# noahpieta/bedops

Measured on AMD Instinct MI355X. Metric: intervals/sec, bedops --intersect 100M×100M BED3 at 1/2/4/8 MI355X, higher is better.
Workload: dtype int64; 1 GPU; bedops --intersect A.bed B.bed: BED3 text in HBM -> parse -> merge -> intersect -> BED text in HBM; parallelism=single GPU, output_rows=38507974

## Files before the change

bedops_amd/csrc/bg_load.hip:

```cpp
#include <algorithm>
#include <cstring>
#include <map>

#include <type_traits>

#include "bg_internal.h"
#include "bg_parse.h"
#include "bg_strtod.h"

#define TT 8192
#define HB 16
#define HA 256
#define LBUF (HB + TT + HA + 32)
#define LCAP 1536
#define REC_CAP (1u << 20)

__device__ __forceinline__ uint32_t nl_mask4(uint32_t w) {
  uint32_t x = w ^ 0x0A0A0A0Au;
  uint32_t nz = ((x & 0x7F7F7F7Fu) + 0x7F7F7F7Fu) | x;
  return ~nz & 0x80808080u;
}

__device__ __forceinline__ uint4 load16(const uint8_t* __restrict__ txt, int64_t base,
                                        uint64_t nbytes) {
// ... 822 lines not shown
    const uint64_t r = r0 + k;
    int64_t key = LLONG_MIN;
    const int64_t le = (k + 1 < L) ? t0 + lst[k + 1] - 1 : last_end;
    if (r < nrows && le >= 0) {
      Fast F;
      const uint32_t run = (rl == rh) ? rl : run_of(R, ls, rl, rh);
      const RunInfo& I = R.info[run];
      double sc = 0;
      if (parse_line_fast(buf, wsm, dgm, lst[k], (uint32_t)(le - ls), F, I.tlen <= 8) &&
          F.toklen == I.tlen && F.tlo == I.tlo && F.thi == I.thi &&
          (kind != BG_BED5 ||
           parse_score_fast(buf, wsm, dgm, lst[k], (uint32_t)(le - ls), F.rest, sc))) {
        emit_row(R, run, ls, r, F.start, F.end, KS, KE, st, key, mlen);
        if (rest_off) {
          rest_off[r] = (uint64_t)(ls + F.rest);
          rest_len[r] = (uint32_t)(le - ls - F.rest);
        }
        if (score) score[r] = sc;
      } else {
        key = PENDING;
      }
    }
    lkey[k] = key;
  }
  for (uint32_t k = threadIdx.x; k < L; k += BG_NT) {
    if (lkey[k] != PENDING) continue;
    lkey[k] = LLONG_MIN;
    const int64_t ls = t0 + lst[k];
    const uint64_t r = r0 + k;
    const int64_t le = (k + 1 < L) ? t0 + lst[k + 1] - 1 : last_end;
    Line Ln;
    parse_line_slow(T, ls, le, kind, Ln);
    if (Ln.err) {
      if (Ln.err == ERR_BLANK) atomicAdd(&st->nblank, 1ULL);
      bg_report(st, r, Ln.err);
      KS[r] = KE[r] = 0;
      continue;
    }
    const uint32_t run = (rl == rh) ? rl : run_of(R, ls, rl, rh);
    if (Ln.hash != R.info[run].hash) {
      bg_report(st, r, ERR_UNSORTED);
      continue;
    }
    int64_t key;
    emit_row(R, run, ls, r, Ln.start, Ln.end, KS, KE, st, key, mlen);
    lkey[k] = key;
    if (rest_off) {
      rest_off[r] = (uint64_t)Ln.rest;
      rest_len[r] = (uint32_t)(le - Ln.rest);
    }
    if (score) {
      score[r] = Ln.score;
      if (Ln.scoreint <= 0) atomicOr(&st->flags, 1ULL);
      if (Ln.scoreint < 0) big_push(st, big, bigcap, r, Ln.spos);
    }
  }
#pragma unroll
  for (int d = 32; d >= 1; d >>= 1) mlen = max(mlen, (int64_t)__shfl_xor(mlen, d, 64));
  if (bg_lane() == 0 && mlen > *(volatile long long*)&st->maxlen) atomicMax(&st->maxlen, (long long)mlen);
  __syncthreads();
  for (uint32_t k = threadIdx.x + 1; k < L; k += BG_NT)
    if (lkey[k] != LLONG_MIN && lkey[k - 1] != LLONG_MIN && lkey[k] < lkey[k - 1])
      bg_report(st, r0 + k, ERR_UNSORTED);
}

__global__ void k_check_bounds(const int64_t* __restrict__ KS, const uint64_t* __restrict__ row0,
                               uint32_t ntiles, uint64_t nrows, bg_dstatus* st) {
  const uint32_t t = blockIdx.x * blockDim.x + threadIdx.x;
  if (t >= ntiles) return;
  const uint64_t r = row0[t];
  for (uint64_t q = r; q < r + 2 && q < nrows; ++q)
    if (q > 0 && KS[q] < KS[q - 1]) bg_report(st, q, ERR_UNSORTED);
}

struct SetTiles {
  int64_t* tmax;
  int64_t* tlast;
  uint64_t* base;
  uint64_t* nloc;
  uint32_t* absorbed;
  uint64_t* nrow;
  int64_t* gb;
};
__device__ __forceinline__ int64_t set_key(const int64_t* X, uint64_t b, int64_t gb, uint64_t i) {
  return gb >= 0 ? (gb | (int64_t)reinterpret_cast<const uint32_t*>(X + b)[i]) : X[b + i];
}

template <bool ONE = false, bool WSO = false, typename BufT = ParseBuf>
__device__ __forceinline__ bool set_row(const BufT& B, const uint16_t* lst, const TileText& T,
                                        const RunTable& R, uint32_t rl, uint32_t rh, int64_t t0,
                                        uint32_t k, uint32_t L, int64_t last_end, int64_t& ks,
                                        int64_t& ke, bg_dstatus* st) {
  const int64_t ls = t0 + lst[k];
  const int64_t le = (k + 1 < L) ? t0 + lst[k + 1] - 1 : last_end;
  if (le < 0) return false;
  const uint32_t run = ONE ? rl : ((rl == rh) ? rl : run_of(R, ls, rl, rh));
  const RunInfo& I = R.info[run];
  uint64_t start, end;
  Fast F;
  bool fast;
  if constexpr (WSO) fast = parse_line_fast_ws(B.buf, B.wsm, lst[k], (uint32_t)(le - ls), F, I.tlen <= 8);
  else fast = parse_line_fast(B.buf, B.wsm, B.dgm, lst[k], (uint32_t)(le - ls), F, I.tlen <= 8);
  if (fast && F.toklen == I.tlen && F.tlo == I.tlo && F.thi == I.thi) {
    start = F.start;
    end = F.end;
  } else {
    Line Ln;
    parse_line_slow(T, ls, le, BG_BED3, Ln);
    if (Ln.err) {
      bg_report(st, 0, Ln.err);
      return false;
    }
    if (Ln.hash != I.hash) {
      bg_report(st, 0, ERR_UNSORTED);
      return false;
    }
    start = Ln.start;
    end = Ln.end;
  }
  if (end > BG_KEY_COORD_MAX || start > end) bg_report(st, 0, ERR_RANGE);
  if (start == end) atomicOr(&st->flags, 2ULL);
  const int64_t g = (int64_t)I.gid << BG_KEY_SHIFT;
  ks = g | (int64_t)(start & BG_COORD_MASK);
  ke = g | (int64_t)(end & BG_COORD_MASK);
  return true;
}

template <int CTRL, int RMASK, bool BC>
__device__ __forceinline__ uint64_t dpp64(uint64_t v) {
  const int lo = __builtin_amdgcn_update_dpp(0, (int)(uint32_t)v, CTRL, RMASK, 0xF, BC);
  const int hi = __builtin_amdgcn_update_dpp(0, (int)(uint32_t)(v >> 32), CTRL, RMASK, 0xF, BC);
  return ((uint64_t)(uint32_t)hi << 32) | (uint32_t)lo;
}
__device__ __forceinline__ uint64_t wave_incl_max_u64(uint64_t v) {
  v = max(v, dpp64<0x111, 0xF, true>(v));
  v = max(v, dpp64<0x112, 0xF, true>(v));
  v = max(v, dpp64<0x114, 0xF, true>(v));
  v = max(v, dpp64<0x118, 0xF, true>(v));
  v = max(v, dpp64<0x142, 0xA, false>(v));
  v = max(v, dpp64<0x143, 0xC, false>(v));
  return v;
}
__device__ __forceinline__ uint64_t wave_shr1_u64(uint64_t v) { return dpp64<0x138, 0xF, true>(v); }

#define BG_SET_OVERFLOW 8ULL
#define BG_ROW_OVERFLOW 16ULL

__device__ __forceinline__ uint32_t wave_incl_max_u32(uint32_t v) {
  v = max(v, dpp32<0x111, 0xF, true>(v));
  v = max(v, dpp32<0x112, 0xF, true>(v));
  v = max(v, dpp32<0x114, 0xF, true>(v));
  v = max(v, dpp32<0x118, 0xF, true>(v));
  v = max(v, dpp32<0x142, 0xA, false>(v));
  v = max(v, dpp32<0x143, 0xC, false>(v));
  return v;
}
__device__ __forceinline__ uint32_t wave_incl_max_v(uint32_t v) { return wave_incl_max_u32(v); }
__device__ __forceinline__ uint64_t wave_incl_max_v(uint64_t v) { return wave_incl_max_u64(v); }
__device__ __forceinline__ uint32_t wave_shr1_v(uint32_t v) { return dpp32<0x138, 0xF, true>(v); }
__device__ __forceinline__ uint64_t wave_shr1_v(uint64_t v) { return wave_shr1_u64(v); }


__device__ __forceinline__ bool parse_score_fast_ws(const uint8_t* buf, const uint32_t* wsm, uint32_t q,
                                                    uint32_t len, uint32_t e1, double& score, bool& isint) {
  uint32_t WS = mask_window(wsm, q + e1);
  const uint32_t l2 = len - e1;
// ... 656 lines not shown
      if (SCORE) ok = ok && le - t0 <= TW + HA_R && score_fast_v(S, q, len, e1, sc);
    }
    if (ok) {
      if (start > end) bg_report(st, r, ERR_RANGE);
      if (start == end) atomicOr(&st->flags, 2ULL);
      mlen = max(mlen, (int64_t)end - (int64_t)start);
      if (ls == pos0) R.row[rl] = r;
      key = gbase | (int64_t)start;
      KS[r] = key;
      KE[r] = gbase | (int64_t)end;
      if (REST) {
        rest_off[r] = (uint64_t)(ls + e1);
        rest_len[r] = len - e1;
      }
      if (SCORE) {
        score[r] = sc;
        nonint |= !isint;
      }
    } else if (live) {
      row_line_general<REST, SCORE>(S, T, R, rl, rh, t0, q, ls, le, r, KS, KE, rest_off, rest_len, score, st,
                                    big, bigcap, key, mlen, nonint);
    }
    const int64_t pk = wave_shr1_i64(key);
    const int64_t prev = lane ? pk : carry;
    if (key != LLONG_MIN && prev != LLONG_MIN && key < prev) bg_report(st, r, ERR_UNSORTED);
    if (j == 0) kf = (int64_t)wave_readlane((uint64_t)key, 0);
    if (j + 1 == rounds) kl = (int64_t)wave_readlane((uint64_t)key, (int)(L - 1 - j * 64));
    carry = (int64_t)wave_readlane((uint64_t)key, 63);
  }
}

template <bool REST, bool SCORE>
__global__ void __launch_bounds__(128) __attribute__((amdgpu_waves_per_eu(6, 8))) k_parse_rv(
    const uint8_t* __restrict__ txt, uint64_t nb, uint64_t nrows, const uint64_t* __restrict__ row0,
    const uint32_t* __restrict__ runlo, const uint32_t* __restrict__ runhi, RunTable R,
    int64_t* __restrict__ KS, int64_t* __restrict__ KE, uint64_t* __restrict__ rest_off,
    uint32_t* __restrict__ rest_len, double* __restrict__ score, bg_dstatus* st, uint64_t* __restrict__ big,
    uint32_t bigcap) {
  __shared__ ParseLdsR SS[2];
  __shared__ uint32_t xl[2];
  __shared__ int64_t xk[2][2];
  const int lane = threadIdx.x & 63, h = __builtin_amdgcn_readfirstlane((int)(threadIdx.x >> 6));
  const uint32_t u = 2 * blockIdx.x + h;
  const int64_t t0 = (int64_t)u * TW;
  const bool inside = (uint64_t)t0 < nb;
  ParseLdsR& S = SS[h];
  int64_t last_end = -1;
  uint32_t L = 0;
  if (inside) {
    SubRegs V;
    load_sub<HA_R>(txt, nb, t0, V);
    L = prologue_v<ParseLdsR, LCAP_R, true, HA_R>(txt, nb, t0, V, S, last_end, st);
  }
  if (lane == 0) xl[h] = L;
  __syncthreads();
  const uint32_t L0 = xl[0];
  if (L0 > LCAP_R || xl[1] > LCAP_R) return;
  const int64_t tt = (int64_t)blockIdx.x * TT;
  const bool has0 = tt == 0 || SS[0].buf[HB - 1] == '\n';
  const uint64_t r0 = row0[blockIdx.x] + (has0 ? 0 : 1) + (h ? L0 : 0);
  int64_t mlen = 0, kf = LLONG_MIN, kl = LLONG_MIN;
  bool nonint = false;
  if (L > 0) {
    const TileText T{txt, S.buf, t0 - HB, t0 + TW + HA_R, nb};
    row_rounds_v<REST, SCORE>(S, T, R, runlo[u], runhi[u], t0, L, last_end, r0, nrows, KS, KE, rest_off,
                              rest_len, score, st, big, bigcap, kf, kl, mlen, nonint);
  }
  if (__ballot(nonint) && lane == 0) atomicOr(&st->flags, 1ULL);
#pragma unroll
  for (int d = 32; d >= 1; d >>= 1) mlen = max(mlen, (int64_t)__shfl_xor(mlen, d, 64));
  if (lane == 0 && mlen > *(volatile long long*)&st->maxlen) atomicMax(&st->maxlen, (long long)mlen);
  if (lane == 0) {
    xk[h][0] = kf;
    xk[h][1] = kl;
  }
  __syncthreads();
  if (h == 1 && lane == 0 && L0 > 0 && L > 0) {
    const int64_t a = xk[0][1], b = xk[1][0];
    if (a != LLONG_MIN && b != LLONG_MIN && b < a) bg_report(st, r0, ERR_UNSORTED);
  }
}


__global__ void __launch_bounds__(BG_NT) k_set_count(const int64_t* __restrict__ LCS, SetTiles TS,
                                                     const int64_t* __restrict__ mex,
                                                     uint32_t ntiles, uint64_t* __restrict__ cnt,
                                                     bg_dstatus* st, uint32_t u0) {
  __shared__ unsigned long long srows[BG_NT / 64];
  const uint32_t t = u0 + blockIdx.x * blockDim.x + threadIdx.x;
  uint64_t rows = 0;
  if (t < ntiles) {
    const uint64_t b = TS.base[t], n = TS.nloc[t];
    const int64_t gb = TS.gb[t];
    rows = TS.nrow[t];
    const int64_t first = n ? set_key(LCS, b, gb, 0) : 0;
    if (n > 0 && t > 0) {
      uint32_t u = t - 1;
      while (u > 0 && TS.tlast[u] == LLONG_MIN) --u;
      if (first < TS.tlast[u]) bg_report(st, 0, ERR_UNSORTED);
    }
    const int64_t M = mex[t];
    uint64_t a = 0;
    if (n && first <= M) {
      uint64_t step = 1;
      while (a + step < n && set_key(LCS, b, gb, a + step) <= M) {
        a += step;
        step <<= 1;
      }
      uint64_t lo = a + 1, hi = min(n, a + step);
      while (lo < hi) {
        const uint64_t mid = (lo + hi) >> 1;
        if (set_key(LCS, b, gb, mid) <= M) lo = mid + 1;
        else hi = mid;
      }
      a = lo;
    }
    TS.absorbed[t] = (uint32_t)a;
    cnt[t] = n - a;
  }
#pragma unroll
  for (int d = 32; d >= 1; d >>= 1) rows += __shfl_xor(rows, d, 64);
  if (bg_lane() == 0) srows[bg_wave()] = rows;
  __syncthreads();
  if (threadIdx.x == 0) {
    unsigned long long r = 0;
    for (int q = 0; q < BG_NT / 64; ++q) r += srows[q];
    if (r) atomicAdd((unsigned long long*)&st->pad[1], r);
  }
}

#define SW_TILES 64
__global__ void __launch_bounds__(BG_NT) k_set_write(const int64_t* __restrict__ LCS,
                                                     const int64_t* __restrict__ LCE, SetTiles TS,
                                                     const int64_t* __restrict__ mex,
                                                     const uint64_t* __restrict__ off,
                                                     uint32_t ntiles, int64_t* __restrict__ CS,
                                                     int64_t* __restrict__ CE, uint32_t u0, uint32_t nlast,
                                                     const uint64_t* __restrict__ carry,
                                                     unsigned long long* __restrict__ total_out) {
  __shared__ uint32_t cpre[SW_TILES + 1];
  __shared__ uint64_t src[SW_TILES], dst[SW_TILES];
  __shared__ uint32_t sab[SW_TILES];
  __shared__ int64_t sgb[SW_TILES];
  __shared__ int64_t first_end[SW_TILES];
  const uint32_t t0 = u0 + blockIdx.x * SW_TILES;
  const uint32_t nt = min((uint32_t)SW_TILES, ntiles - t0);
  const uint64_t cy = carry ? *carry : 0;
  uint32_t c = 0;
  if (threadIdx.x < nt) {
    const uint32_t t = t0 + threadIdx.x;
    const uint64_t b = TS.base[t], n = TS.nloc[t], a = TS.absorbed[t];
    const int64_t M = mex[t], gb = TS.gb[t];
    c = (uint32_t)(n - a);
    src[threadIdx.x] = b;
    sab[threadIdx.x] = (uint32_t)a;
    sgb[threadIdx.x] = gb;
    dst[threadIdx.x] = cy + off[t];
    first_end[threadIdx.x] = (c > 0) ? max(M, a > 0 ? set_key(LCE, b, gb, a - 1) : LLONG_MIN) : 0;
    if (t + 1 == nlast) {
      const uint64_t total = cy + off[t] + c;
      if (total > 0) CE[total - 1] = max(M, TS.tmax[t]);
      if (total_out) *total_out = total;
    }
  }
  if (threadIdx.x < 64) {
    const uint32_t inc = wave_incl_scan(c, OpSum());
    cpre[threadIdx.x + 1] = inc;
    if (threadIdx.x == 0) cpre[0] = 0;
  }
  __syncthreads();
  const uint32_t tot = cpre[nt];
  for (uint32_t e = threadIdx.x; e < tot; e += BG_NT) {
    uint32_t lo = 0, hi = nt - 1;
    while (lo < hi) {
      const uint32_t mid = (lo + hi + 1) >> 1;
      if (cpre[mid] <= e) lo = mid;
      else hi = mid - 1;
    }
    const uint32_t j = e - cpre[lo];
    const uint64_t g = dst[lo] + j, b = src[lo], i = sab[lo] + j;
    const int64_t gb = sgb[lo];
    CS[g] = set_key(LCS, b, gb, i);
    if (g > 0) CE[g - 1] = j == 0 ? first_end[lo] : set_key(LCE, b, gb, i - 1);
  }
}

constexpr uint32_t BK_T = 4096;

__global__ void __launch_bounds__(BG_NT) k_blank_marks(const uint8_t* __restrict__ txt, uint64_t nb,
                                                       uint32_t nt, int64_t* __restrict__ tnl,
                                                       int64_t* __restrict__ tns) {
  const uint32_t lane = threadIdx.x & 63, t = blockIdx.x * (BG_NT / 64) + (threadIdx.x >> 6);
  if (t >= nt) return;
  const uint64_t b0 = (uint64_t)t * BK_T + 64ull * lane;
  int64_t lnl = -1, lns = -2;
  for (uint32_t k = 0; k < 64 && b0 + k < nb; ++k) {
    const uint8_t ch = txt[b0 + k];
    if (ch == '\n') lnl = (int64_t)(b0 + k);
    else if (!bg_isws(ch)) lns = (int64_t)(b0 + k);
  }
  for (int d = 32; d >= 1; d >>= 1) {
    lnl = max(lnl, (int64_t)__shfl_xor(lnl, d, 64));
    lns = max(lns, (int64_t)__shfl_xor(lns, d, 64));
  }
  if (lane == 0) {
    tnl[t] = lnl;
    tns[t] = lns;
  }
}

__global__ void __launch_bounds__(BG_NT) k_blank_pack(const uint8_t* __restrict__ txt, uint64_t nb,
                                                      uint32_t nt, const int64_t* __restrict__ xnl,
                                                      const int64_t* __restrict__ xns,
                                                      uint64_t* __restrict__ cnt,
                                                      const uint64_t* __restrict__ off,
                                                      uint8_t* __restrict__ out) {
  const uint32_t lane = threadIdx.x & 63, t = blockIdx.x * (BG_NT / 64) + (threadIdx.x >> 6);
  if (t >= nt) return;
  const uint64_t b0 = (uint64_t)t * BK_T + 64ull * lane;
  int64_t lnl = -1, lns = -2;
  for (uint32_t k = 0; k < 64 && b0 + k < nb; ++k) {
    const uint8_t ch = txt[b0 + k];
    if (ch == '\n') lnl = (int64_t)(b0 + k);
    else if (!bg_isws(ch)) lns = (int64_t)(b0 + k);
  }
  for (int d = 1; d < 64; d <<= 1) {
    const int64_t a = __shfl_up(lnl, d, 64), b = __shfl_up(lns, d, 64);
    if (lane >= (uint32_t)d) {
      lnl = max(lnl, a);
      lns = max(lns, b);
    }
  }
  int64_t cnl = __shfl_up(lnl, 1, 64), cns = __shfl_up(lns, 1, 64);
  if (lane == 0) cnl = -1, cns = -2;
  cnl = max(cnl, xnl[t]);
  cns = max(cns, xns[t]);
  const int64_t snl = cnl, sns = cns;
  uint32_t keep = 0;
  for (uint32_t k = 0; k < 64 && b0 + k < nb; ++k) {
    const uint8_t ch = txt[b0 + k];
    const bool sp = ch == '\n' || bg_isws(ch);
    keep += !(sp && cnl > cns);
    if (ch == '\n') cnl = (int64_t)(b0 + k);
    else if (!sp) cns = (int64_t)(b0 + k);
  }
  uint32_t pre = keep;
  for (int d = 1; d < 64; d <<= 1) {
    const uint32_t a = __shfl_up(pre, d, 64);
    if (lane >= (uint32_t)d) pre += a;
  }
  if (!out) {
    if (lane == 63) cnt[t] = pre;
    return;
  }
  uint64_t o = off[t] + pre - keep;
  cnl = snl;
  cns = sns;
  for (uint32_t k = 0; k < 64 && b0 + k < nb; ++k) {
    const uint8_t ch = txt[b0 + k];
    const bool sp = ch == '\n' || bg_isws(ch);
    if (!(sp && cnl > cns)) out[o++] = ch;
    if (ch == '\n') cnl = (int64_t)(b0 + k);
    else if (!sp) cns = (int64_t)(b0 + k);
// ... 17 lines not shown
  uint64_t* tot = (uint64_t*)(w + 4ull * nt);
  int rc = 0;
  if (nt) {
    const dim3 g(bg_blocks(nt, BG_NT / 64));
    BG_LAUNCH(c, "k_blank_marks", k_blank_marks, g, dim3(BG_NT), txt, nb, nt, tnl, tns);
    rc = bg_hip_ok(c, hipGetLastError());
    if (!rc) rc = bg_scan_max_i64(c, tnl, xnl, nt, -1);
    if (!rc) rc = bg_scan_max_i64(c, tns, xns, nt, -2);
    if (!rc) {
      BG_LAUNCH(c, "k_blank_pack", k_blank_pack, g, dim3(BG_NT), txt, nb, nt, (const int64_t*)xnl,
                (const int64_t*)xns, cnt, (const uint64_t*)nullptr, (uint8_t*)nullptr);
      rc = bg_hip_ok(c, hipGetLastError());
    }
    if (!rc) rc = bg_scan_sum_u64(c, cnt, cnt, nt, tot);
    if (!rc) {
      BG_LAUNCH(c, "k_blank_pack", k_blank_pack, g, dim3(BG_NT), txt, nb, nt, (const int64_t*)xnl,
                (const int64_t*)xns, (uint64_t*)nullptr, (const uint64_t*)cnt, (uint8_t*)o);
      rc = bg_hip_ok(c, hipGetLastError());
    }
    if (!rc) rc = bg_fetch_u64(c, tot, nout);
  }
  bg_release(c, w);
  if (rc) {
    bg_release(c, o);
    *nout = 0;
    return rc;
  }
  *out = o;
  return 0;
}

static const char* kind_name(int k) {
  return (k == BG_BED5 || k == BG_BED5_REST) ? "BED5" : (k == BG_BED3_REST ? "BED3+rest" : "BED3");
}

static int report_status(bg_ctx* c, int file, const bg_dstatus& h) {
  if (h.first_bad == ~0ULL) return 0;
  uint64_t row = h.first_bad >> 8;
  int code = (int)(h.first_bad & 0xff);
  char msg[256];
  const char* what = "";
  int rc = BG_E_PARSE;
  switch (code) {
    case ERR_PARSE: what = "malformed BED line (expected: chrom<tab>start<tab>end...)"; break;
    case ERR_CHROM: what = "chromosome name longer than 127 characters"; rc = BG_E_CHROM; break;
    case ERR_RANGE: what = "coordinate out of range (end < start or >= 2^40)"; rc = BG_E_RANGE; break;
    case ERR_UNSORTED: what = "input is not sorted (use sort-bed)"; rc = BG_E_UNSORTED; break;
    case ERR_BLANK: what = "blank line inside the data is not supported by the GPU loader"; rc = BG_E_BLANK; break;
    case ERR_SCORE: what = "score column is not a plain decimal number"; rc = BG_E_UNSUPPORTED; break;
  }
  snprintf(msg, sizeof(msg), "input %d, data line %llu: %s", file + 1,
           (unsigned long long)row + 1, what);
  return bg_fail(c, rc, msg);
}

struct LoadState {
  const uint8_t* txt = nullptr;
  uint64_t nb = 0;
  uint32_t ntiles = 0;
  uint32_t rc = 0;
  uint64_t* row0 = nullptr;
  uint64_t* cnt = nullptr;
  int64_t* fls = nullptr;
  uint64_t* fhash = nullptr;
  uint32_t* fnl = nullptr;
  uint32_t* blist = nullptr;
  RunRec* recs = nullptr;
  std::vector<int64_t> run_pos;
  std::vector<uint64_t> run_hash;
  const RunRec* hrec = nullptr;
  uint32_t nrec = 0;
  uint64_t* hrow = nullptr;
  std::vector<RunInfo> info;
  RunInfo* d_info = nullptr;
  uint64_t* d_row = nullptr;
  uint32_t* rlo = nullptr;
  uint32_t* rhi = nullptr;
  uint32_t nrows_run = 0;
  int64_t* lcs = nullptr;
  int64_t* lce = nullptr;
  int64_t* tmax = nullptr;
  int64_t* tlast = nullptr;
  int64_t* mex = nullptr;
  int64_t* sex = nullptr;
  uint64_t* tbase = nullptr;
  uint64_t* nloc = nullptr;
  uint64_t* tcnt = nullptr;
  uint32_t* absorbed = nullptr;
  int64_t* tgb = nullptr;
  uint32_t set_nt = 0;
  uint64_t* big = nullptr;
  uint32_t bigcap = 0;
  bool blank = false;
};

static void release_state(bg_ctx* c, LoadState& S) {
  for (void* p : {(void*)S.row0, (void*)S.cnt, (void*)S.fls, (void*)S.fhash, (void*)S.fnl,
                  (void*)S.blist, (void*)S.recs,
                  (void*)S.d_info, (void*)S.d_row, (void*)S.rlo, (void*)S.rhi, (void*)S.lcs,
                  (void*)S.lce, (void*)S.tmax, (void*)S.tlast, (void*)S.mex, (void*)S.sex,
                  (void*)S.tbase, (void*)S.nloc, (void*)S.tcnt, (void*)S.absorbed,
                  (void*)S.tgb, (void*)S.big})
    bg_release(c, p);
  S = LoadState();
}

static int side_begin(bg_ctx* c, hipStream_t& main) {
  if (!c->sstream) {
    if (hipStreamCreateWithFlags(&c->sstream, hipStreamNonBlocking) != hipSuccess ||
        hipEventCreateWithFlags(&c->sfork, hipEventDisableTiming) != hipSuccess ||
        hipEventCreateWithFlags(&c->sjoin, hipEventDisableTiming) != hipSuccess) {
      (void)hipGetLastError();
      return bg_fail(c, BG_E_HIP, "side stream creation failed");
    }
  }
  BG_HIP(c, hipEventRecord(c->sfork, c->stream));
  BG_HIP(c, hipStreamWaitEvent(c->sstream, c->sfork, 0));
  c->defer_release = true;
  main = c->stream;
  c->stream = c->sstream;
  return 0;
}
static void side_end(bg_ctx* c, hipStream_t main) {
  (void)hipEventRecord(c->sjoin, c->sstream);
  c->stream = main;
}
static int side_join(bg_ctx* c) {
  if (!c->defer_release) return 0;
  int rc = bg_hip_ok(c, hipStreamWaitEvent(c->stream, c->sjoin, 0));
  c->defer_release = false;
  for (auto& b : c->deferred) c->free_list.push_back(b);
  c->deferred.clear();
  return rc;
}

static int scout_pass(bg_ctx* c, LoadState& S, uint64_t* ctr) {
  const uint32_t nt = S.ntiles;
  BG_LAUNCH(c, "k_scout", k_scout, dim3(bg_blocks(nt, SCOUT_TILES)), dim3(BG_NT), S.txt, S.nb, nt,
            S.cnt, S.fnl);
  BG_HIP(c, hipGetLastError());
  return bg_scan_sum_u64(c, S.cnt, S.row0, nt, &ctr[0]);
}

static int scout_one(bg_ctx* c, const bg_input& in, bg_table* T, LoadState& S, uint64_t* ctr) {
  T->kind = in.kind;
  const uint8_t* txt;
  if (in.on_device) {
    if (((uintptr_t)in.data & 15) != 0) return bg_fail(c, BG_E_ARG, "device text must be 16-byte aligned");
    txt = (const uint8_t*)in.data;
  } else {
    T->own_text = (char*)bg_alloc(c, in.nbytes + 16);
    if (!T->own_text) return BG_E_NOMEM;
    if (in.nbytes)
      BG_HIP(c, hipMemcpyAsync(T->own_text, in.data, in.nbytes, hipMemcpyHostToDevice, c->stream));
    txt = (const uint8_t*)T->own_text;
  }
  T->text = (const char*)txt;
  T->nbytes = in.nbytes;
  S.txt = txt;
  S.nb = in.nbytes;
  S.ntiles = in.nbytes ? bg_blocks(in.nbytes, TT) : 0;
  if (S.ntiles == 0) return 0;
  const uint32_t nt = S.ntiles;
  S.rc = (uint32_t)std::min<uint64_t>(REC_CAP, (uint64_t)nt * (TT / 6 + 2) + 16);
  const bool set = in.kind == BG_BED3_SET;
  const bool scout = !set;
  if (scout) {
    S.row0 = (uint64_t*)bg_alloc(c, 8ull * nt);
    S.cnt = (uint64_t*)bg_alloc(c, 8ull * nt);
    S.fnl = (uint32_t*)bg_alloc(c, 4ull * nt);
    if (!S.row0 || !S.cnt || !S.fnl) return BG_E_NOMEM;
  }
  S.fls = (int64_t*)bg_alloc(c, 8ull * nt);
  S.fhash = (uint64_t*)bg_alloc(c, 8ull * nt);
  S.blist = (uint32_t*)bg_alloc(c, 4ull * nt);
  S.recs = (RunRec*)bg_alloc(c, sizeof(RunRec) * (size_t)S.rc);
  if (!S.fls || !S.fhash || !S.blist || !S.recs)
    return BG_E_NOMEM;
  if (scout) {
    int rc = scout_pass(c, S, ctr);
    if (rc) return rc;
  }
  BG_LAUNCH(c, "k_tokhash", k_tokhash, dim3(bg_blocks(nt, 256)), dim3(256), txt, S.nb, nt, scout ? S.fnl : nullptr,
// ... 80 lines not shown
  else
    BG_LAUNCH(c, "k_run_range", k_run_range<TW>, dim3(bg_blocks(ntr, 256)), dim3(256), R, ntr, S.rlo, S.rhi);
  BG_HIP(c, hipGetLastError());
  return 0;
}

static int parse_one(bg_ctx* c, const bg_input& in, bg_table* T, LoadState& S,
                     const std::map<std::string, int32_t>& gid, bg_dstatus* st) {
  const uint64_t na = T->n ? T->n : 1;
  T->ks = (int64_t*)bg_alloc(c, 8 * na);
  T->ke = (int64_t*)bg_alloc(c, 8 * na);
  if (!T->ks || !T->ke) return BG_E_NOMEM;
  if (in.kind == BG_BED3_REST || in.kind == BG_BED5_REST) {
    T->rest_off = (uint64_t*)bg_alloc(c, 8 * na);
    T->rest_len = (uint32_t*)bg_alloc(c, 4 * na);
    if (!T->rest_off || !T->rest_len) return BG_E_NOMEM;
  }
  if (in.kind == BG_BED5 || in.kind == BG_BED5_REST) {
    T->score = (double*)bg_alloc(c, 8 * na);
    if (!T->score) return BG_E_NOMEM;
  }
  const uint32_t nr = (uint32_t)S.run_pos.size();
  if (S.ntiles == 0 || T->n == 0 || nr == 0) return 0;
  const bool rv = !c->row_wide;
  RunTable R;
  int rc = upload_runs(c, T, S, gid, R, rv ? TW : TT);
  if (rc) return rc;
  if (T->score) {
    static const uint64_t cap0 = [] {
      const char* e = getenv("BEDGPU_BIGCAP");
      return e ? (uint64_t)std::max(1, atoi(e)) : (uint64_t)(1u << 20);
    }();
    S.bigcap = (uint32_t)std::min<uint64_t>(T->n, std::max<uint64_t>(cap0, c->big_need));
    S.big = (uint64_t*)bg_alloc(c, 16ull * (S.bigcap ? S.bigcap : 1));
    if (!S.big) return BG_E_NOMEM;
  }
  const int kind = in.kind == BG_BED5_REST ? BG_BED5 : in.kind;
  if (rv) {
#define BG_ROWV(RE, SC)                                                                                    \
  BG_LAUNCH(c, "k_parse", (k_parse_rv<RE, SC>), dim3(S.ntiles), dim3(128), S.txt, S.nb, T->n, S.row0, S.rlo, \
            S.rhi, R, T->ks, T->ke, T->rest_off, T->rest_len, T->score, st, S.big, S.bigcap)
    const bool re = T->rest_off != nullptr, sc = kind == BG_BED5;
    if (re && sc) BG_ROWV(true, true);
    else if (re) BG_ROWV(true, false);
    else if (sc) BG_ROWV(false, true);
    else BG_ROWV(false, false);
#undef BG_ROWV
  } else {
    BG_LAUNCH(c, "k_parse_wide", k_parse, dim3(S.ntiles), dim3(BG_NT), S.txt, S.nb, T->n, S.row0, S.rlo, S.rhi,
              kind, R, T->ks, T->ke, T->rest_off, T->rest_len, T->score, st, S.big, S.bigcap);
  }
  BG_HIP(c, hipGetLastError());
  BG_LAUNCH(c, "k_check_bounds", k_check_bounds, dim3(bg_blocks(S.ntiles, 256)), dim3(256), T->ks,
            S.row0, S.ntiles, T->n, st);
  BG_HIP(c, hipGetLastError());
  S.nrows_run = nr;
  return 0;
}

static int parse_set_one(bg_ctx* c, bg_table* T, LoadState& S,
                         const std::map<std::string, int32_t>& gid, bg_dstatus* st) {
  T->is_set = true;
  const uint32_t nr = (uint32_t)S.run_pos.size();
  const uint32_t nt = (uint32_t)bg_blocks(S.nb, (uint64_t)TW);
  const uint64_t cap = nt ? (uint64_t)nt * SCAP_W : 1;
  T->cs = (int64_t*)bg_alloc(c, 8 * cap);
  T->ce = (int64_t*)bg_alloc(c, 8 * cap);
  if (!T->cs || !T->ce) return BG_E_NOMEM;
  if (nt == 0 || nr == 0) return 0;
  RunTable R;
  int rc = upload_runs(c, T, S, gid, R, TW);
  if (rc) return rc;
  S.lcs = (int64_t*)bg_alloc(c, 8 * cap);
  S.lce = (int64_t*)bg_alloc(c, 8 * cap);
  S.tmax = (int64_t*)bg_alloc(c, 8ull * nt);
  S.tlast = (int64_t*)bg_alloc(c, 8ull * nt);
  S.mex = (int64_t*)bg_alloc(c, 8ull * nt);
  S.tbase = (uint64_t*)bg_alloc(c, 8ull * nt);
  S.nloc = (uint64_t*)bg_alloc(c, 8ull * nt);
  S.tcnt = (uint64_t*)bg_alloc(c, 8ull * nt);
  S.absorbed = (uint32_t*)bg_alloc(c, 4ull * nt);
  S.tgb = (int64_t*)bg_alloc(c, 8ull * nt);
  S.cnt = (uint64_t*)bg_alloc(c, 8ull * nt);
  if (!S.lcs || !S.lce || !S.tmax || !S.tlast || !S.mex || !S.tbase || !S.nloc ||
      !S.tcnt || !S.absorbed || !S.cnt || !S.tgb)
    return BG_E_NOMEM;
  SetTiles TS{S.tmax, S.tlast, S.tbase, S.nloc, S.absorbed, S.cnt, S.tgb};
  BG_LAUNCH(c, "k_parse_set", k_parse_set_v, dim3(nt), dim3(64), S.txt, S.nb, nt, S.rlo, S.rhi, R,
            S.lcs, S.lce, TS, st);
  BG_HIP(c, hipGetLastError());
  S.set_nt = nt;
  return 0;
}

static int set_merge_count(bg_ctx* c, LoadState& S, bg_dstatus* st) {
  const uint32_t nt = S.set_nt;
  SetTiles TS{S.tmax, S.tlast, S.tbase, S.nloc, S.absorbed, S.cnt, S.tgb};
  int rc;
  if ((rc = bg_scan_max_i64(c, S.tmax, S.mex, nt, LLONG_MIN))) return rc;
  BG_LAUNCH(c, "k_set_count", k_set_count, dim3(bg_blocks(nt, BG_NT)), dim3(BG_NT), S.lcs, TS,
            (const int64_t*)S.mex, nt, S.tcnt, st, 0u);
  BG_HIP(c, hipGetLastError());
  return bg_scan_sum_u64(c, S.tcnt, S.tcnt, nt, (uint64_t*)&st->pad[0]);
}
static int set_merge_write(bg_ctx* c, bg_table* T, LoadState& S) {
  const uint32_t nt = S.set_nt;
  S.set_nt = 0;
  SetTiles TS{S.tmax, S.tlast, S.tbase, S.nloc, S.absorbed, S.cnt, S.tgb};
  BG_LAUNCH(c, "k_set_write", k_set_write, dim3(bg_blocks(nt, SW_TILES)), dim3(BG_NT), S.lcs,
            S.lce, TS, (const int64_t*)S.mex, (const uint64_t*)S.tcnt, nt, T->cs, T->ce, 0u, nt,
            (const uint64_t*)nullptr, (unsigned long long*)nullptr);
  BG_HIP(c, hipGetLastError());
  return 0;
}
static int parse_set_merge(bg_ctx* c, bg_table* T, LoadState& S, bg_dstatus* st) {
  const int rc = set_merge_count(c, S, st);
  return rc ? rc : set_merge_write(c, T, S);
}

static int set_merge_side(bg_ctx* c, bg_table* T, LoadState& S, bg_dstatus* st, bool write) {
  hipStream_t main;
  int rc = side_begin(c, main);
  if (rc) return rc;
  rc = write ? set_merge_write(c, T, S) : set_merge_count(c, S, st);
  side_end(c, main);
  return rc;
}

static int finish_one(bg_ctx* c, int idx, const bg_input& in, bg_table* T, LoadState& S,
                      const bg_dstatus& h) {
  T->run_row0.assign(1, 0);
  if (T->is_set) {
    T->n = h.pad[1];
    T->nc = h.pad[0];
    T->has_zero_len = (h.flags & 2ULL) != 0;
    T->run_row0.push_back(T->n);
    if (S.ntiles == 0 || T->n == 0) T->run_name.clear();
    return 0;
  }
  if (S.ntiles == 0 || T->n == 0 || S.run_pos.empty()) {
    T->run_name.clear();
    return 0;
  }
  int rc = report_status(c, idx, h);
  if (rc) return rc;
  if (h.nbig) {
    if (h.nbig > S.bigcap || !T->score)
      return bg_fail(c, BG_E_UNSUPPORTED, "too many scores needing the exact big-number conversion");
    BG_LAUNCH(c, "k_score_big", k_score_big, dim3(bg_blocks(h.nbig, 64)), dim3(64), S.txt, S.nb, S.big, h.nbig,
              T->score);
    rc = bg_hip_ok(c, hipGetLastError());
    if (rc) return rc;
  }
  if ((in.kind == BG_BED5 || in.kind == BG_BED5_REST) && (h.flags & 1ULL)) T->score_int = false;
  T->has_zero_len = (h.flags & 2ULL) != 0;
  T->maxlen = h.maxlen;
  uint32_t nkeep = S.hrow ? S.nrows_run : 0;
  while (nkeep > 0 && S.hrow[nkeep - 1] == ~0ULL) --nkeep;
  T->run_name.resize(nkeep);
  T->run_row0.clear();
  for (uint32_t k = 0; k < nkeep; ++k) T->run_row0.push_back(S.hrow[k]);
  T->run_row0.push_back(T->n);
  return 0;
}

static int build_dictionary(bg_ctx* c, bg_set* s, std::map<std::string, int32_t>& gid,
                            std::string& packed, std::vector<uint32_t>& off,
                            std::vector<uint32_t>& len) {
  std::vector<std::string> all;
  for (bg_table* T : s->t)
    for (auto& nm : T->run_name) all.push_back(nm);
  std::sort(all.begin(), all.end(),
            [](const std::string& a, const std::string& b) { return strcmp(a.c_str(), b.c_str()) < 0; });
  all.erase(std::unique(all.begin(), all.end()), all.end());
  if (all.size() >= (1u << 22)) return bg_fail(c, BG_E_UNSUPPORTED, "too many chromosomes");
  s->names = all;
  for (size_t k = 0; k < all.size(); ++k) gid[all[k]] = (int32_t)k;
  off.assign(all.size() + 1, 0);
  len.assign(all.size() + 1, 0);
  for (size_t k = 0; k < all.size(); ++k) {
    off[k] = (uint32_t)packed.size();
    len[k] = (uint32_t)all[k].size();
    s->max_name_len = std::max<uint32_t>(s->max_name_len, len[k]);
    packed += all[k];
  }
  const size_t nbn = (packed.size() + 16) & ~(size_t)15, nbo = 4 * off.size(), blk = nbn + 2 * nbo;
  s->d_names = (char*)bg_alloc(c, blk);
  if (!s->d_names) return BG_E_NOMEM;
  s->d_name_off = (uint32_t*)(s->d_names + nbn);
  s->d_name_len = (uint32_t*)(s->d_names + nbn + nbo);
  char* h = (char*)bg_pin_take(c, blk);
  std::vector<char> hv;
  if (!h) {
    hv.resize(blk);
// ... 228 lines not shown
```

Before: 63.75 billion intervals/s.

## Fuse set-merge max scan and count sum scan into grouped kernels

Replaces the generic device-wide max scan and sum scan around the set-merge count with a small group-level scheme. Per-group maxima are reduced first, k_set_count computes the exclusive running max inline and emits per-group kept counts, a single-block kernel scans those group sums, and k_set_write rebuilds each tile offset from the group prefix plus in-group counts. This is meant to cut kernel launches and the multi-pass scan traffic. In exchange, each count block loops over all previous group maxima and the group scan runs in a single block.

Result: no change. 63.47 billion intervals/s (-0.4%).

```diff
diff --git a/bedops_amd/csrc/bg_load.hip b/bedops_amd/csrc/bg_load.hip
--- a/bedops_amd/csrc/bg_load.hip
+++ b/bedops_amd/csrc/bg_load.hip
@@ -928,6 +928,7 @@
   uint64_t* nrow;
   int64_t* gb;
 };
+#define SET_G BG_NT
 __device__ __forceinline__ int64_t set_key(const int64_t* X, uint64_t b, int64_t gb, uint64_t i) {
   return gb >= 0 ? (gb | (int64_t)reinterpret_cast<const uint32_t*>(X + b)[i]) : X[b + i];
 }
@@ -1750,14 +1751,42 @@
 }
 
 
+__global__ void __launch_bounds__(BG_NT) k_set_gmax(const int64_t* __restrict__ tmax, uint32_t ntiles,
+                                                    int64_t* __restrict__ gmax) {
+  __shared__ int64_t sh[BG_NT / 64];
+  const uint32_t t = blockIdx.x * SET_G + threadIdx.x;
+  int64_t m = t < ntiles ? tmax[t] : (int64_t)LLONG_MIN;
+#pragma unroll
+  for (int d = 32; d >= 1; d >>= 1) m = max(m, (int64_t)__shfl_xor(m, d, 64));
+  if (bg_lane() == 0) sh[bg_wave()] = m;
+  __syncthreads();
+  if (threadIdx.x == 0) {
+#pragma unroll
+    for (int q = 1; q < BG_NT / 64; ++q) m = max(m, sh[q]);
+    gmax[blockIdx.x] = m;
+  }
+}
+
 __global__ void __launch_bounds__(BG_NT) k_set_count(const int64_t* __restrict__ LCS, SetTiles TS,
-                                                     const int64_t* __restrict__ mex,
-                                                     uint32_t ntiles, uint64_t* __restrict__ cnt,
-                                                     bg_dstatus* st, uint32_t u0) {
-  __shared__ unsigned long long srows[BG_NT / 64];
-  const uint32_t t = u0 + blockIdx.x * blockDim.x + threadIdx.x;
-  uint64_t rows = 0;
+                                                     const int64_t* __restrict__ gmax,
+                                                     int64_t* __restrict__ mex, uint32_t ntiles,
+                                                     uint64_t* __restrict__ cnt,
+                                                     uint64_t* __restrict__ gsum, bg_dstatus* st) {
+  __shared__ unsigned long long srows[BG_NT / 64], scnt[BG_NT / 64];
+  __shared__ int64_t scar[BG_NT / 64], shm[BG_NT / 64 + 1];
+  const uint32_t t = blockIdx.x * SET_G + threadIdx.x;
+  int64_t cm = LLONG_MIN;
+  for (uint32_t g = threadIdx.x; g < blockIdx.x; g += BG_NT) cm = max(cm, gmax[g]);
+#pragma unroll
+  for (int d = 32; d >= 1; d >>= 1) cm = max(cm, (int64_t)__shfl_xor(cm, d, 64));
+  if (bg_lane() == 0) scar[bg_wave()] = cm;
+  int64_t gtot;
+  int64_t M = block_excl_scan(t < ntiles ? TS.tmax[t] : (int64_t)LLONG_MIN, OpMax(), (int64_t)LLONG_MIN, shm, &gtot);
+#pragma unroll
+  for (int q = 0; q < BG_NT / 64; ++q) M = max(M, scar[q]);
+  uint64_t rows = 0, kept = 0;
   if (t < ntiles) {
+    mex[t] = M;
     const uint64_t b = TS.base[t], n = TS.nloc[t];
     const int64_t gb = TS.gb[t];
     rows = TS.nrow[t];
@@ -1767,7 +1796,6 @@
       while (u > 0 && TS.tlast[u] == LLONG_MIN) --u;
       if (first < TS.tlast[u]) bg_report(st, 0, ERR_UNSORTED);
     }
-    const int64_t M = mex[t];
     uint64_t a = 0;
     if (n && first <= M) {
       uint64_t step = 1;
@@ -1784,37 +1812,79 @@
       a = lo;
     }
     TS.absorbed[t] = (uint32_t)a;
-    cnt[t] = n - a;
+    cnt[t] = kept = n - a;
   }
 #pragma unroll
-  for (int d = 32; d >= 1; d >>= 1) rows += __shfl_xor(rows, d, 64);
-  if (bg_lane() == 0) srows[bg_wave()] = rows;
+  for (int d = 32; d >= 1; d >>= 1) {
+    rows += __shfl_xor(rows, d, 64);
+    kept += __shfl_xor(kept, d, 64);
+  }
+  if (bg_lane() == 0) {
+    srows[bg_wave()] = rows;
+    scnt[bg_wave()] = kept;
+  }
   __syncthreads();
   if (threadIdx.x == 0) {
-    unsigned long long r = 0;
-    for (int q = 0; q < BG_NT / 64; ++q) r += srows[q];
+    unsigned long long r = 0, k = 0;
+    for (int q = 0; q < BG_NT / 64; ++q) {
+      r += srows[q];
+      k += scnt[q];
+    }
     if (r) atomicAdd((unsigned long long*)&st->pad[1], r);
-  }
+    gsum[blockIdx.x] = k;
+  }
+}
+
+#define GS_ITEMS 8
+__global__ void __launch_bounds__(BG_NT) k_set_gscan(uint64_t* __restrict__ gsum, uint32_t ng,
+                                                     unsigned long long* __restrict__ total) {
+  __shared__ uint64_t sh[BG_NT / 64 + 1];
+  uint64_t run = 0;
+  for (uint32_t b0 = 0; b0 < ng; b0 += BG_NT * GS_ITEMS) {
+    const uint32_t i0 = b0 + threadIdx.x * GS_ITEMS;
+    uint64_t x[GS_ITEMS], s = 0;
+#pragma unroll
+    for (int k = 0; k < GS_ITEMS; ++k) {
+      x[k] = i0 + k < ng ? gsum[i0 + k] : 0;
+      s += x[k];
+    }
+    uint64_t tot;
+    uint64_t pre = run + block_excl_scan(s, OpSum(), (uint64_t)0, sh, &tot);
+#pragma unroll
+    for (int k = 0; k < GS_ITEMS; ++k) {
+      if (i0 + k < ng) gsum[i0 + k] = pre;
+      pre += x[k];
+    }
+    run += tot;
+  }
+  if (threadIdx.x == 0) *total = run;
 }
 
 #define SW_TILES 64
 __global__ void __launch_bounds__(BG_NT) k_set_write(const int64_t* __restrict__ LCS,
                                                      const int64_t* __restrict__ LCE, SetTiles TS,
                                                      const int64_t* __restrict__ mex,
-                                                     const uint64_t* __restrict__ off,
+                                                     const uint64_t* __restrict__ cnt,
+                                                     const uint64_t* __restrict__ gsum,
                                                      uint32_t ntiles, int64_t* __restrict__ CS,
-                                                     int64_t* __restrict__ CE, uint32_t u0, uint32_t nlast,
-                                                     const uint64_t* __restrict__ carry,
-                                                     unsigned long long* __restrict__ total_out) {
+                                                     int64_t* __restrict__ CE) {
   __shared__ uint32_t cpre[SW_TILES + 1];
-  __shared__ uint64_t src[SW_TILES], dst[SW_TILES];
+  __shared__ uint64_t src[SW_TILES];
+  __shared__ uint64_t spre[BG_NT / 64];
   __shared__ uint32_t sab[SW_TILES];
   __shared__ int64_t sgb[SW_TILES];
   __shared__ int64_t first_end[SW_TILES];
-  const uint32_t t0 = u0 + blockIdx.x * SW_TILES;
+  static_assert(SET_G % SW_TILES == 0 && SET_G <= BG_NT, "a workgroup's tiles lie in one group");
+  const uint32_t t0 = blockIdx.x * SW_TILES;
   const uint32_t nt = min((uint32_t)SW_TILES, ntiles - t0);
-  const uint64_t cy = carry ? *carry : 0;
+  const uint32_t g0 = t0 / SET_G * SET_G;
+  uint64_t before = threadIdx.x < t0 - g0 ? cnt[g0 + threadIdx.x] : 0;
+#pragma unroll
+  for (int d = 32; d >= 1; d >>= 1) before += __shfl_xor(before, d, 64);
+  if (bg_lane() == 0) spre[bg_wave()] = before;
   uint32_t c = 0;
+  int64_t fin = LLONG_MIN;
+  const bool fin_tile = threadIdx.x < nt && t0 + threadIdx.x + 1 == ntiles;
   if (threadIdx.x < nt) {
     const uint32_t t = t0 + threadIdx.x;
     const uint64_t b = TS.base[t], n = TS.nloc[t], a = TS.absorbed[t];
@@ -1823,13 +1893,8 @@
     src[threadIdx.x] = b;
     sab[threadIdx.x] = (uint32_t)a;
     sgb[threadIdx.x] = gb;
-    dst[threadIdx.x] = cy + off[t];
     first_end[threadIdx.x] = (c > 0) ? max(M, a > 0 ? set_key(LCE, b, gb, a - 1) : LLONG_MIN) : 0;
-    if (t + 1 == nlast) {
-      const uint64_t total = cy + off[t] + c;
-      if (total > 0) CE[total - 1] = max(M, TS.tmax[t]);
-      if (total_out) *total_out = total;
-    }
+    if (fin_tile) fin = max(M, TS.tmax[t]);
   }
   if (threadIdx.x < 64) {
     const uint32_t inc = wave_incl_scan(c, OpSum());
@@ -1837,7 +1902,11 @@
     if (threadIdx.x == 0) cpre[0] = 0;
   }
   __syncthreads();
+  uint64_t dst = gsum[t0 / SET_G];
+#pragma unroll
+  for (int q = 0; q < BG_NT / 64; ++q) dst += spre[q];
   const uint32_t tot = cpre[nt];
+  if (fin_tile && dst + tot > 0) CE[dst + tot - 1] = fin;
   for (uint32_t e = threadIdx.x; e < tot; e += BG_NT) {
     uint32_t lo = 0, hi = nt - 1;
     while (lo < hi) {
@@ -1846,7 +1915,7 @@
       else hi = mid - 1;
     }
     const uint32_t j = e - cpre[lo];
-    const uint64_t g = dst[lo] + j, b = src[lo], i = sab[lo] + j;
+    const uint64_t g = dst + e, b = src[lo], i = sab[lo] + j;
     const int64_t gb = sgb[lo];
     CS[g] = set_key(LCS, b, gb, i);
     if (g > 0) CE[g - 1] = j == 0 ? first_end[lo] : set_key(LCE, b, gb, i - 1);
@@ -2030,7 +2099,8 @@
   int64_t* tmax = nullptr;
   int64_t* tlast = nullptr;
   int64_t* mex = nullptr;
-  int64_t* sex = nullptr;
+  int64_t* gmax = nullptr;
+  uint64_t* gsum = nullptr;
   uint64_t* tbase = nullptr;
   uint64_t* nloc = nullptr;
   uint64_t* tcnt = nullptr;
@@ -2046,7 +2116,7 @@
   for (void* p : {(void*)S.row0, (void*)S.cnt, (void*)S.fls, (void*)S.fhash, (void*)S.fnl,
                   (void*)S.blist, (void*)S.recs,
                   (void*)S.d_info, (void*)S.d_row, (void*)S.rlo, (void*)S.rhi, (void*)S.lcs,
-                  (void*)S.lce, (void*)S.tmax, (void*)S.tlast, (void*)S.mex, (void*)S.sex,
+                  (void*)S.lce, (void*)S.tmax, (void*)S.tlast, (void*)S.mex, (void*)S.gmax, (void*)S.gsum,
                   (void*)S.tbase, (void*)S.nloc, (void*)S.tcnt, (void*)S.absorbed,
                   (void*)S.tgb, (void*)S.big})
     bg_release(c, p);
@@ -2293,8 +2363,10 @@
   S.absorbed = (uint32_t*)bg_alloc(c, 4ull * nt);
   S.tgb = (int64_t*)bg_alloc(c, 8ull * nt);
   S.cnt = (uint64_t*)bg_alloc(c, 8ull * nt);
+  S.gmax = (int64_t*)bg_alloc(c, 8ull * bg_blocks(nt, SET_G));
+  S.gsum = (uint64_t*)bg_alloc(c, 8ull * bg_blocks(nt, SET_G));
   if (!S.lcs || !S.lce || !S.tmax || !S.tlast || !S.mex || !S.tbase || !S.nloc ||
-      !S.tcnt || !S.absorbed || !S.cnt || !S.tgb)
+      !S.tcnt || !S.absorbed || !S.cnt || !S.tgb || !S.gmax || !S.gsum)
     return BG_E_NOMEM;
   SetTiles TS{S.tmax, S.tlast, S.tbase, S.nloc, S.absorbed, S.cnt, S.tgb};
   BG_LAUNCH(c, "k_parse_set", k_parse_set_v, dim3(nt), dim3(64), S.txt, S.nb, nt, S.rlo, S.rhi, R,
@@ -2307,20 +2379,23 @@
 static int set_merge_count(bg_ctx* c, LoadState& S, bg_dstatus* st) {
   const uint32_t nt = S.set_nt;
   SetTiles TS{S.tmax, S.tlast, S.tbase, S.nloc, S.absorbed, S.cnt, S.tgb};
-  int rc;
-  if ((rc = bg_scan_max_i64(c, S.tmax, S.mex, nt, LLONG_MIN))) return rc;
-  BG_LAUNCH(c, "k_set_count", k_set_count, dim3(bg_blocks(nt, BG_NT)), dim3(BG_NT), S.lcs, TS,
-            (const int64_t*)S.mex, nt, S.tcnt, st, 0u);
+  const uint32_t ng = bg_blocks(nt, SET_G);
+  BG_LAUNCH(c, "k_set_gmax", k_set_gmax, dim3(ng), dim3(BG_NT), (const int64_t*)S.tmax, nt, S.gmax);
   BG_HIP(c, hipGetLastError());
-  return bg_scan_sum_u64(c, S.tcnt, S.tcnt, nt, (uint64_t*)&st->pad[0]);
+  BG_LAUNCH(c, "k_set_count", k_set_count, dim3(ng), dim3(BG_NT), S.lcs, TS, (const int64_t*)S.gmax,
+            S.mex, nt, S.tcnt, S.gsum, st);
+  BG_HIP(c, hipGetLastError());
+  BG_LAUNCH(c, "k_set_gscan", k_set_gscan, dim3(1), dim3(BG_NT), S.gsum, ng, &st->pad[0]);
+  BG_HIP(c, hipGetLastError());
+  return 0;
 }
 static int set_merge_write(bg_ctx* c, bg_table* T, LoadState& S) {
   const uint32_t nt = S.set_nt;
   S.set_nt = 0;
   SetTiles TS{S.tmax, S.tlast, S.tbase, S.nloc, S.absorbed, S.cnt, S.tgb};
   BG_LAUNCH(c, "k_set_write", k_set_write, dim3(bg_blocks(nt, SW_TILES)), dim3(BG_NT), S.lcs,
-            S.lce, TS, (const int64_t*)S.mex, (const uint64_t*)S.tcnt, nt, T->cs, T->ce, 0u, nt,
-            (const uint64_t*)nullptr, (unsigned long long*)nullptr);
+            S.lce, TS, (const int64_t*)S.mex, (const uint64_t*)S.tcnt,
+            (const uint64_t*)S.gsum, nt, T->cs, T->ce);
   BG_HIP(c, hipGetLastError());
   return 0;
 }
```
